# tangtang888/video-edge-ai-proxy

Measured on AMD Instinct MI355X. Metric: decoded FPS (whole node) + p50 VideoLatestImage latency, 256×1080p RTSP, higher is better.
Workload: dtype uint8 (BGR24 frames; bf16-capable consumer path)

## Files before the change

csrc/bind_codec.cpp:

```cpp
#include "bind_common.h"
#include "vep/avc.h"
#include "vep/codec.h"
#include "vep/hevc_dec.h"
#include "vep/hevc_kern.h"
#include "vep/synth.h"

struct CpuDecoder {
  StreamParser parser;
  MbUpdate upd;
  HostSurface surf;
  PictureInfo last;
  avc::Decoder avc;
  std::vector<HostSurface> slots;
  bool general = false;
  int target = 0;
  int coded = 0;
  bool fields_out = false;
  HostSurface woven;
  mutable HostSurface weave_tmp;
  const HostSurface& out() const { return general ? (fields_out ? woven : slots[size_t(target)]) : surf; }
  const HostSurface& frame_of(const avc::OutFrame& f) const {
    if (!f.fields) return slots[size_t(f.slot)];
    avc::weave_fields(slots[2 * size_t(f.slot)], slots[2 * size_t(f.slot) + 1], weave_tmp);
    return weave_tmp;
// ... 209 lines not shown
      .def_readwrite("weighted_b", &avc::AvcHighConfig::weighted_b)
      .def_readwrite("direct_spatial", &avc::AvcHighConfig::direct_spatial)
      .def_readwrite("scaling", &avc::AvcHighConfig::scaling)
      .def_readwrite("slices", &avc::AvcHighConfig::slices)
      .def_readwrite("deblock_idc", &avc::AvcHighConfig::deblock_idc)
      .def_readwrite("chroma_qp_offset", &avc::AvcHighConfig::chroma_qp_offset)
      .def_readwrite("second_chroma_qp_offset", &avc::AvcHighConfig::second_chroma_qp_offset)
      .def_readwrite("coverage", &avc::AvcHighConfig::coverage)
      .def_readwrite("interlaced", &avc::AvcHighConfig::interlaced)
      .def_readwrite("mono", &avc::AvcHighConfig::mono)
      .def_readwrite("fields", &avc::AvcHighConfig::fields)
      .def_readwrite("marking", &avc::AvcHighConfig::marking)
      .def_readwrite("objects", &avc::AvcHighConfig::objects)
      .def_readwrite("noise", &avc::AvcHighConfig::noise)
      .def_readwrite("temporal_noise", &avc::AvcHighConfig::temporal_noise)
      .def_readwrite("seed", &avc::AvcHighConfig::seed);
  py::class_<avc::AvcHighEncoder>(m, "AvcHighEncoder")
      .def(py::init<const avc::AvcHighConfig&>())
      .def("next", &avc::AvcHighEncoder::next, py::call_guard<py::gil_scoped_release>())
      .def("picture", [](const avc::AvcHighEncoder& e) { return surface_planes(e.reconstruction()); })
      .def("source", [](const avc::AvcHighEncoder& e) { return surface_planes(e.source()); })
      .def_property_readonly("last_pts", &avc::AvcHighEncoder::last_pts)
      .def_property_readonly("last_type", [](const avc::AvcHighEncoder& e) { return std::string(1, e.last_type()); })
      .def_property_readonly("last_display_index", &avc::AvcHighEncoder::last_display_index)
      .def_property_readonly("sps_nal", [](const avc::AvcHighEncoder& e) { return to_bytes(e.sps_nal().data(), e.sps_nal().size()); })
      .def_property_readonly("pps_nal", [](const avc::AvcHighEncoder& e) { return to_bytes(e.pps_nal().data(), e.pps_nal().size()); });

  py::class_<hevc::HevcEncConfig>(m, "HevcEncConfig")
      .def(py::init<>())
      .def_readwrite("width", &hevc::HevcEncConfig::width)
// ... 211 lines not shown
```

csrc/bind_codec_hooks.cpp:

```cpp
#include "bind_common.h"
#include "vep/avc.h"
#include "vep/avc_cavlc.h"
#include "vep/avc_recon.h"
#include "vep/cabac.h"
#include "vep/codec.h"
#include "vep/h264.h"
#include "vep/hevc_ctu.h"
#include "vep/hevc_dec.h"
#include "vep/hevc_kern.h"
#include "vep/synth.h"

struct XorShift {
  u64 x;
  XorShift(u64 seed, u64 salt) : x(seed * 0x9E3779B97F4A7C15ull + salt) {}
  u64 operator()() { return x ^= x << 13, x ^= x >> 7, x ^= x << 17; }
};

static std::vector<u8> rbsp_of(const std::string& nal) {
  std::vector<u8> r(nal.size());
  r.resize(ebsp_to_rbsp(reinterpret_cast<const u8*>(nal.data()), nal.size(), r.data()));
  return r;
}

void bind_codec_hooks(py::module_& m) {
// ... 317 lines not shown
      mbs += p->mbs.size();
      coefs += p->coefs.size();
      mvs += p->mvs.size();
      for (const avc::MbRec& m : p->mbs)
        if (m.kind != avc::kIPcm) nz += avc::coef_values(p->coefs.data(), m);
    }
    py::gil_scoped_acquire g;
    py::dict d;
    d["pictures"] = pics;
    d["mbs"] = mbs;
    d["coefs"] = coefs;
    d["nonzero"] = nz;
    d["mvs"] = mvs;
    return d;
  });
  m.def("hevc_record_stats", [](const std::vector<std::shared_ptr<AccessUnit>>& aus) {
    py::gil_scoped_release r;
    hevc::Decoder dec;
    dec.set_gpu_mode(true);
    u64 pics = 0, tus = 0, coefs = 0, nz = 0, pus = 0;
    for (const auto& au : aus) {
      dec.decode(*au);
      for (const auto& p : dec.take_gpu_pictures()) {
        ++pics;
        tus += p->tus.size();
        pus += p->pus.size();
        coefs += p->coefs.size();
        for (i16 c : p->coefs) nz += c != 0;
      }
    }
// ... 135 lines not shown
```

csrc/vep/avc.cpp:

```cpp
#include "avc.h"

#include <immintrin.h>

#include <algorithm>
#include <array>

#include "avc_cavlc.h"
#include "avc_internal.h"
#include "fanout.h"

namespace vep::avc {

using h264::Pps;
using h264::Sps;


void MbNeighbours::reset(int wmbs, int hmbs, bool ring) {
  w_ = wmbs;
  h_ = hmbs;
  cur_ = -1;
  run_slice_ = ~0u;
  run_start_ = 0;
  announced_ = 0;
  const size_t n = size_t(wmbs) * hmbs;
// ... 1402 lines not shown
      pi.coded_height = sps.coded_height();
      pi.width = sps.width();
      pi.height = sps.height();
      pi.crop_left = sps.crop_left;
      pi.crop_top = sps.crop_top;
      pi.pict_type = "PBISi"[sh.type()];
      pi.idr = sh.idr();
      pi.frame_num = sh.frame_num;
      pi.fps = sps.fps();
      pic->au.pts = au.pts;
      pic->au.dts = au.dts;
      pic->au.arrival_ms = au.arrival_ms;
      pic->au.keyframe = au.keyframe;
      pic->au.corrupt = au.corrupt;
      pic->au.tag = tag;
      nb_.reset(W, Hp, true);
      if (sh.field_pic) {
        const int fs = second_field ? pair_.slot : pick_slot();
        pic->target = 2 * fs + int(sh.bottom_field);
        if (!second_field) {
          pair_ = OpenPair{};
          pair_.open = true;
          pair_.slot = fs;
          pair_.frame_num = sh.frame_num;
          pair_.bottom = int(sh.bottom_field);
          pair_.ref = sh.nal_ref_idc != 0;
          pair_.boundary = sh.idr();
          pair_.hard = sh.idr() && (hard_flush || reorder_cur_ == 0);
          pair_.f.slot = fs;
          pair_.f.info = pic->info;
          pair_.f.au = pic->au;
// ... 322 lines not shown

void ColBuild::none(int mb) {
  const int per = col->corners ? 4 : 16;
  ColMotion::Blk* out = &col->b[size_t(mb) * size_t(per)];
  for (int k = 0; k < per; ++k) out[k] = ColMotion::Blk{{0, 0}, 0u, i8(-1)};
}

void ColBuild::store(int mb, const MbState& st) {
  if (is_intra(st.kind) || !uids) {
    none(mb);
    return;
  }
  static constexpr u8 kCorner[4] = {0, 3, 12, 15};
  const auto& lu = *uids;
  if (col->corners) {
    ColMotion::Blk out[4];
    for (int k = 0; k < 4; ++k) {
      const int l = st.ref[0][k] >= 0 ? 0 : 1;
      const int ri = st.ref[l][k];
      out[k] = ri < 0 ? ColMotion::Blk{{0, 0}, 0u, i8(-1)}
                      : ColMotion::Blk{{st.mv[l][kCorner[k]][0], st.mv[l][kCorner[k]][1]}, uid_tab[l][ri & 31], i8(ri)};
    }
    stream_words(&col->b[size_t(mb) * 4], out, sizeof out);
    return;
  }
  ColMotion::Blk* out = &col->b[size_t(mb) * 16];
  for (int blk = 0; blk < 16; ++blk) {
    const int b8 = ((blk >> 3) << 1) | ((blk & 3) >> 1);
    const int l = st.ref[0][b8] >= 0 ? 0 : 1;
    const int ri = st.ref[l][b8];
    if (ri < 0) {
      out[blk] = ColMotion::Blk{{0, 0}, 0u, i8(-1)};
      continue;
    }
    out[blk] = ColMotion::Blk{{st.mv[l][blk][0], st.mv[l][blk][1]},
                              size_t(ri) < lu[size_t(l)].size() ? lu[size_t(l)][size_t(ri)] : 0u, i8(ri)};
  }
}

std::shared_ptr<ColMotion> build_col_motion(const MbNeighbours& nb, int wmbs, int hmbs,
                                            const std::vector<std::array<std::vector<u32>, 2>>& slice_uids,
                                            bool corners, Recycler<ColMotion>* pool) {
  auto col = pool ? pool->acquire([](ColMotion&) {}) : std::make_shared<ColMotion>();
  col->wmbs = wmbs;
  col->hmbs = hmbs;
  col->corners = corners;
  const int per = corners ? 4 : 16;
  col->b.resize(size_t(wmbs) * hmbs * size_t(per));
  static constexpr u8 kCorner[4] = {0, 3, 12, 15};
  for (int mb = 0; mb < wmbs * hmbs; ++mb) {
    const MbState& st = nb.at(mb);
    ColMotion::Blk* out = &col->b[size_t(mb) * size_t(per)];
// ... 214 lines not shown
  const __m256i tl = _mm256_setr_epi32(0, 0, 2, 2, 0, 0, 2, 2);
  const u32 all = u32(_mm256_movemask_epi8(_mm256_and_si256(_mm256_cmpeq_epi32(a, v0), _mm256_cmpeq_epi32(b, v0))));
  const u32 q8 = u32(_mm256_movemask_epi8(_mm256_and_si256(_mm256_cmpeq_epi32(a, _mm256_permutevar8x32_epi32(a, tl)),
                                                           _mm256_cmpeq_epi32(b, _mm256_permutevar8x32_epi32(b, tl)))));
  return (all == 0xFFFFFFFFu ? 1u : 0u) | (q8 == 0xFFFFFFFFu ? 2u : 0u);
#else
  u32 v[16];
  std::memcpy(v, mv, sizeof v);
  bool u16 = true, u8x8 = true;
  for (int b = 1; b < 16; ++b) u16 &= v[b] == v[0];
  for (int b = 0; b < 16; ++b) u8x8 &= v[b] == v[((b >> 3) << 3) | (b & 2)];
  return (u16 ? 1u : 0u) | (u8x8 ? 2u : 0u);
#endif
}

static inline void store_motion(Picture& pic, MbRec& m, const MbState& s) {
  const int nl = (m.flags & kMbL1) ? 2 : 1;
  u32 u = 3;
  for (int l = 0; l < nl; ++l) u &= motion_uniformity(&s.mv[l][0][0]);
  m.flags |= (u & 1) ? kMbMv16 : ((u & 2) ? kMbMv8x8 : 0);
  m.mv = u32(pic.mvs.size());
  const int per = (u & 1) ? 2 : ((u & 2) ? 8 : 32);
  i16* out = pic.mvs.extend(size_t(per * nl));
  for (int l = 0; l < nl; ++l, out += per) {
    const i16* v = &s.mv[l][0][0];
    if (per == 2) {
      std::memcpy(out, v, 4);
    } else if (per == 8) {
      std::memcpy(out, v, 4);
      std::memcpy(out + 2, v + 4, 4);
      std::memcpy(out + 4, v + 16, 4);
      std::memcpy(out + 6, v + 20, 4);
    } else {
      std::memcpy(out, v, 64);
    }
  }
}

static inline void store_rec(MbRec* dst, const MbRec& m) {
  static_assert(sizeof(MbRec) % 8 == 0 && sizeof(ColMotion::Blk) * 4 % 8 == 0, "8-byte words");
  stream_words(dst, &m, sizeof(MbRec));
}

void store_skip_mb(Picture& pic, int mb, MbRec& m, const MbState& s) {
  m.coef = u32(pic.coefs.size());
  m.luma_coded = 0;
  m.chroma_coded = 0;
  m.wp = 0;
  m.res = kNoRes;
  store_motion(pic, m, s);
  ++pic.inter_mbs;
  if (!(m.dbk & 1)) pic.deblock = true;
  for (int k = 0; k < 4; ++k) {
    const int r0 = m.ref[k], r1 = m.ref1[k];
    VEP_CHECK((r0 != 0xFF || r1 != 0xFF) && (r0 == 0xFF || r0 < pic.dpb_slots) && (r1 == 0xFF || r1 < pic.dpb_slots) &&
                  (r1 == 0xFF || (m.flags & kMbL1)),
              "skipped macroblock reference slot outside the DPB");
  }
  VEP_CHECK(m.qp <= 51 + pic.qp_bias && m.qpc <= 51 + pic.qpc_bias && m.qpc2 <= 51 + pic.qpc_bias,
            "macroblock QP out of range");
  store_rec(&pic.mbs[size_t(mb)], m);
  if (pic.colb) pic.colb->store(mb, s);
}

void store_mb(Picture& pic, int mb, MbRec m, const MbState& s, const MbResidual* res, const u8* pcm,
              const WpEntry* wp) {
  m.coef = u32(pic.coefs.size());
  m.luma_coded = 0;
  m.chroma_coded = 0;
  if (m.kind == kIPcm) {
    VEP_CHECK(pcm, "I_PCM macroblock without samples");
    const size_t ns = pic.cf == 2 ? size_t(kPcmMaxSamples) : size_t(kPcmMbBytes);
    const size_t o = pic.coefs.size(), nb = pic.bd > 8 ? 2 * ns : ns;
    pic.coefs.resize(o + nb / 2);
    std::memcpy(pic.coefs.data() + o, pcm, nb);
  } else if (res && (res->luma | res->chroma)) {
    m.luma_coded = res->luma;
    m.chroma_coded = res->chroma;
    if (res->t8) m.flags |= kMbT8x8;
    const i16* grp[32];
    int ng = 0;
// ... 10 lines not shown
    for (int g = 0; g < ng; ++g) {
      mask[g] = nonzero_mask16(grp[g]);
      nv += __builtin_popcount(mask[g]);
    }
    const size_t o = pic.coefs.size();
    i16* out = pic.coefs.extend(size_t(ng + nv) + 8);
    std::memcpy(out, mask, size_t(ng) * sizeof(u16));
    i16* v = out + ng;
    for (int g = 0; g < ng; ++g) v = compact16(grp[g], mask[g], v);
    pic.coefs.resize(o + size_t(ng + nv));
  }
  m.mv = 0;
  m.wp = 0;
  m.flags &= u8(~(kMbMv8x8 | kMbMv16));
  if (m.kind == kSkip || m.kind == kInter) {
    store_motion(pic, m, s);
    if (wp && (m.flags & kMbWp)) {
      m.wp = u32(pic.wps.size());
      pic.wps.insert(pic.wps.end(), wp, wp + 4);
    } else {
      m.flags &= u8(~kMbWp);
    }
    ++pic.inter_mbs;
  } else if (m.kind == kIPcm) {
    ++pic.inter_mbs;
  } else {
    ++pic.intra_mbs;
  }
  m.res = is_intra(m.kind) && m.kind != kIPcm && (m.luma_coded | m.chroma_coded) ? u32(pic.intra_res++) : kNoRes;
  if (!(m.dbk & 1)) pic.deblock = true;
  validate_written_mb(pic, m);
// ... 356 lines not shown
```

csrc/vep/avc.h:

```cpp
#pragma once

#include <array>
#include <map>
#include <memory>

#include "hostmem.h"
#include "recycle.h"
#include "avc_recon.h"
#include "codec.h"

namespace vep::avc {

constexpr int kMaxDpbSlots = 34;

struct AuMeta {
  i64 pts = 0, dts = 0, arrival_ms = 0;
  i64 tag = 0;
  bool keyframe = false, corrupt = false;
};

struct OutFrame {
  int slot = -1;
  PictureInfo info;
  AuMeta au;
// ... 324 lines not shown
    return corners ? size_t(mb) * 4 + size_t(((blk >> 3) << 1) | ((blk & 3) >> 1)) : size_t(mb) * 16 + size_t(blk);
  }
};

struct ColBuild {
  ColMotion* col = nullptr;
  const std::array<std::vector<u32>, 2>* uids = nullptr;
  u32 uid_tab[2][32] = {};
  void set_uids(const std::array<std::vector<u32>, 2>* u) {
    uids = u;
    for (int l = 0; l < 2; ++l)
      for (size_t k = 0; k < 32; ++k) uid_tab[l][k] = u && k < (*u)[size_t(l)].size() ? (*u)[size_t(l)][k] : 0u;
  }
  void store(int mb, const MbState& st);
  void none(int mb);
};

struct RefPic {
  int slot = -1;
  int frame_num = 0;
  int frame_num_wrap = 0;
  bool long_term = false;
  int lt_idx = 0;
  int poc = 0;
  u32 uid = 0;
  std::shared_ptr<const ColMotion> col;
  u8 fields = 3;
  u8 lt_fields = 0;
  int poc_f[2] = {0, 0};
  u32 uid_f[2] = {0, 0};
// ... 55 lines not shown
  int cf_ = 1;
  bool have_idr_ = false;
  int pinned_slot_ = -1;
  int last_out_poc_ = 0;
  i64 last_out_epoch_ = -1;
  u32 epoch_ = 0;
  int adaptive_reorder_ = 0;
  int reorder_cur_ = 0;
  u32 next_uid_ = 1;
  int prev_poc_msb_ = 0, prev_poc_lsb_ = 0;
  int prev_frame_num_ = 0, prev_frame_num_offset_ = 0;
  bool prev_ref_mmco5_ = false;
  std::vector<std::vector<MbState>> spare_;
  struct SliceUnit;
  bool parallel_slices_ = true;
  std::vector<std::unique_ptr<SliceUnit>> units_;
  u64 parallel_slices_run_ = 0;
  bool field_mode_ = false;
  struct OpenPair {
    bool open = false;
    int slot = -1, frame_num = 0, bottom = 0;
    int poc[2] = {0, 0};
    bool ref = false, boundary = false, hard = false;
    u8 have = 0;
    OutFrame f;
  } pair_;
  void close_pair(Picture& pic);

 public:
  Decoder();
  ~Decoder();
  u64 parallel_slices_run() const { return parallel_slices_run_; }
  u64 mmco_ops[7] = {0, 0, 0, 0, 0, 0, 0};
  u64 list_mods = 0, long_term_marked = 0;
  u64 redundant_slices_skipped = 0;
};

void cpu_reconstruct(const Picture& pic, std::vector<HostSurface>& slots);
void weave_fields(const HostSurface& top, const HostSurface& bottom, HostSurface& frame);

struct MbLevels {
  int luma[16][16];
  int dc[16];
  int cdc[2][4];
  int cac[2][4][16];
  u16 lmask = 0;
  u8 cmask = 0;
// ... 9 lines not shown
      for (int b = 0; b < 4; ++b) {
        if (cdc[c][b]) dcmask |= u8(2 << c);
        for (int k = 0; k < 16; ++k)
          if (cac[c][b][k]) cmask |= u8(1u << (c * 4 + b));
      }
  }
};
struct MbResidual {
  i16 blk[32][16];
  i16 b8[4][64];
  u16 luma = 0;
  u16 chroma = 0;
  bool t8 = false;
};
void dequantize_mb(const MbLevels& lv, bool i16x16, int qp, int qpc, MbResidual& out);
void store_mb(Picture& pic, int mb, MbRec m, const MbState& s, const MbResidual* res, const u8* pcm,
              const WpEntry* wp = nullptr);
void store_skip_mb(Picture& pic, int mb, MbRec& m, const MbState& s);
void cpu_reconstruct_mb(const Picture& pic, int mb, std::vector<HostSurface>& slots);
void cpu_deblock(const Picture& pic, HostSurface& target);
void intra4x4_neighbours(const Picture& pic, int mb, int idx, const HostSurface& T, Intra4Nb& n);
void intra16_neighbours(const Picture& pic, int mb, const HostSurface& T, Intra16Nb& n);
void chroma_neighbours(const Picture& pic, int mb, int c, const HostSurface& T, IntraChromaNb& n);
void intra8x8_neighbours(const Picture& pic, int mb, int q, const HostSurface& T, int* f, bool& has_top,
                         bool& has_left);

class StreamEncoder {
 public:
  virtual ~StreamEncoder() = default;
  virtual std::shared_ptr<AccessUnit> next() = 0;
  virtual const HostSurface& reconstruction() const = 0;
  virtual const HostSurface& source() const = 0;
  virtual i64 last_pts() const = 0;
// ... 53 lines not shown
  int weighted_b = 0;
  bool direct_spatial = true;
  bool scaling = false;
  int slices = 1;
  int deblock_idc = 0;
  int chroma_qp_offset = 0, second_chroma_qp_offset = 0;
  bool coverage = false;
  bool interlaced = false;
  bool marking = false;
  bool fields = false;
  bool mono = false;
  int bit_depth = 8;
  int chroma_format = 1;
  int objects = 3;
  double noise = 3.0, temporal_noise = 0.0;
  u64 seed = 1;
};

class AvcHighEncoder : public StreamEncoder {
 public:
  explicit AvcHighEncoder(const AvcHighConfig& cfg);
  ~AvcHighEncoder() override;
  std::shared_ptr<AccessUnit> next() override;
  const HostSurface& reconstruction() const override;
  const HostSurface& source() const override;
  i64 last_pts() const override;
  i64 last_display_index() const;
  char last_type() const;
  const AvcHighConfig& config() const { return cfg_; }
  const std::vector<u8>& sps_nal() const override;
// ... 10 lines not shown
```

csrc/vep/avc_enc_high.cpp:

```cpp
#include <cmath>
#include <deque>
#include <map>

#include "avc.h"
#include "avc_internal.h"
#include "avc_scene.h"
#include "h264.h"

namespace vep::avc {

namespace {

struct Idct8Inverse {
  double inv[8][8];
  Idct8Inverse() {
    double m[8][8];
    for (int k = 0; k < 8; ++k) {
      int x[8] = {0, 0, 0, 0, 0, 0, 0, 0};
      x[k] = 1024;
      idct8_1d(x);
      for (int i = 0; i < 8; ++i) m[i][k] = x[i] / 1024.0;
    }
    double a[8][16];
    for (int i = 0; i < 8; ++i)
// ... 76 lines not shown
    int lt_idx = 0;
    u8 lt_fields = 0;
  };
  int max_lt_idx = -1;
  std::vector<Ref> dpb;
  struct Job {
    i64 disp;
    int type;
    bool ref;
    bool idr;
    int parity = -1;
  };
  std::deque<Job> plan;
  std::map<i64, HostSurface> sources;
  i64 next_disp = 0, gop_start = 0, rendered = -1, coded = 0;
  int prev_ref_fn = 0, idr_id = -1;
  u32 next_uid = 1;
  Picture pic;
  MbNeighbours nb;
  HostSurface recon, src_out;
  i64 last_disp = 0, last_pts = 0;
  char last_type = 'I';
  const HostSurface* cur_src = nullptr;
  bool fields = false;
  int ph = 0;
  HostSurface field_src;
  int pair_slot = -1, pair_fn = 0;
  int bd = 8, qpbd = 0;
  int cf = 1;
  const u8* scan4 = kZigzag4x4;
// ... 53 lines not shown
    pps.cabac = c.cabac;
    pps.bottom_field_pic_order = c.interlaced;
    pps.weighted_pred = c.weighted_p;
    pps.weighted_bipred_idc = c.weighted_b;
    pps.chroma_qp_index_offset = c.chroma_qp_offset;
    pps.second_chroma_qp_index_offset = c.second_chroma_qp_offset;
    pps.deblocking_filter_control = true;
    pps.transform_8x8_mode = c.t8x8;
    pps.scaling.flat();
    auto nal = [](const std::vector<u8>& rbsp, std::vector<u8>& out) { rbsp_to_ebsp(rbsp.data(), rbsp.size(), out); };
    nal(h264::write_sps(sps), sps_nal);
    nal(h264::write_pps(pps), pps_nal);
    ph = fields ? hpx / 2 : hpx;
    slots.resize((size_t(sps.max_num_ref_frames) + 2) * (fields ? 2 : 1));
    for (auto& s : slots) s.alloc(wpx, ph, bd, cf);
    scene.make(SceneConfig{c.width, c.height, wpx, hpx, c.objects, c.noise, c.temporal_noise, c.seed}, rng);
  }

  bool is_idr_pos(i64 d) const { return d == 0 || (d + cfg.idr_phase) % cfg.gop == 0; }

  const HostSurface& source_of(i64 d) {
    while (rendered < d) {
      ++rendered;
      if (rendered > 0) scene.advance();
      scene.render();
      scene.add_sensor_noise(rendered);
      if (bd > 8 || cf == 2) {
        HostSurface& w = sources[rendered];
        const HostSurface& s8 = scene.src;
        w.alloc(s8.coded_w, s8.coded_h, bd, cf);
        const int sh = bd - 8;
// ... 826 lines not shown
    const double dist = (e.poc - env.cur_poc) / 2.0;
    const int mx = mb % W, my = mb / W;
    auto cost = [&](int vx, int vy) {
      int s = 0;
      for (int i = 0; i < 16; i += 2)
        for (int j = 0; j < 16; j += 2) {
          const int x = mx * 16 + j, y = my * 16 + i;
          const int p = bd > 8 ? luma_qpel(R.y16.data(), wpx, wpx, ph, x + (vx >> 2), y + (vy >> 2), vx & 3, vy & 3, bd)
                               : luma_qpel(R.y.data(), wpx, wpx, ph, x + (vx >> 2), y + (vy >> 2), vx & 3, vy & 3);
          s += std::abs(S(x, y) - p);
        }
      return s * 4 + 4 * (std::abs(vx - pmv[0]) + std::abs(vy - pmv[1]));
    };
    std::vector<std::pair<int, int>> cand = {{0, 0}, {pmv[0], pmv[1]}};
    const double ys = fields ? 0.5 : 1.0;
    for (const Scene::Obj& o : scene.objs) {
      if (o.x > mx * 16 + 24 || o.x + o.w < mx * 16 - 8 || o.y * ys > my * 16 + 24 || (o.y + o.h) * ys < my * 16 - 8)
        continue;
      cand.push_back({int(std::lround(o.vx * 4 * dist)), int(std::lround(o.vy * ys * 4 * dist))});
    }
    best_sad = 1 << 30;
    for (auto [vx, vy] : cand) {
      const int c = cost(vx, vy);
      if (c < best_sad) {
        best_sad = c;
        best[0] = vx;
        best[1] = vy;
      }
    }
    for (int step : {4, 2, 1}) {
// ... 634 lines not shown
```

csrc/vep/avc_mb.cpp:

```cpp
#include <algorithm>
#include <memory>
#include <cstddef>
#include <cstring>

#include "avc_cabac.h"
#include "avc_cavlc.h"
#include "avc_internal.h"

namespace vep::avc {

namespace {

struct Dequant {
  int ls4[6][6][16];
  int ls8[2][6][64];
  explicit Dequant(const h264::ScalingLists& sl) {
    for (int l = 0; l < 6; ++l)
      for (int m = 0; m < 6; ++m)
        for (int k = 0; k < 16; ++k) {
          const int pos = kZigzag4x4[k];
          ls4[l][m][pos] = int(sl.l4[l][k]) * norm_adjust(m, pos >> 2, pos & 3);
        }
    for (int l = 0; l < 2; ++l)
      for (int m = 0; m < 6; ++m)
// ... 112 lines not shown
    auto cond = [&](int m) { return m >= 0 && !nb_.at(m).skip ? 1 : 0; };
    const int inc = cond(nb_.mb_at(mb, -1, 0)) + cond(nb_.mb_at(mb, 0, -1));
    return bins->mb_skip(type_ == h264::kB, inc, v) != 0;
  }

  void skip_mb(int mb, bool fresh) {
    MbState& s = nb_.at(mb);
    if (fresh) {
      s = MbState{};
      s.slice = u16(env_.slice);
      nb_.begin(mb);
    }
    s.kind = kSkip;
    s.skip = 1;
    s.qp = u8(qp_ + qpbd_);
    MbResidual res;
    res.luma = 0;
    res.chroma = 0;
    if (type_ == h264::kP) {
      s.ref[0][0] = s.ref[0][1] = s.ref[0][2] = s.ref[0][3] = 0;
      need_ref(0, 0);
      int mv[2];
      nb_.pskip_mv(mb, mv);
      for (auto& v : s.mv[0]) {
        v[0] = i16(mv[0]);
        v[1] = i16(mv[1]);
      }
    } else {
      s.direct16 = 1;
      s.direct8 = 0xF;
      if (fast_direct_) direct16_spatial(mb, s);
      else direct(mb, s, 0xF);
    }
    prev_qpd_nz = 0;
    if (!weighted_ && !kWrite) emit_skip(mb, s);
    else emit(mb, s, res, 0, 0, nullptr);
  }

  void coded_mb(int mb, bool fresh) {
    MbState& s = nb_.at(mb);
    if (fresh) {
      s = MbState{};
      s.slice = u16(env_.slice);
      nb_.begin(mb);
    } else if constexpr (!kWrite) {
      std::memset(static_cast<void*>(s.mv), 0, sizeof s.mv);
    }
    int mbt = read_mb_type(mb, kWrite ? want->mb_type : 0);
    int itype = -1;
    if (type_ == h264::kI) {
      itype = mbt;
// ... 587 lines not shown
          const int tx = (16384 + std::abs(td / 2)) / td;
          const int dsf = clip3i(-1024, 1023, (tb * tx + 32) >> 6);
          for (int k = 0; k < 2; ++k) {
            m0[k] = (dsf * mvc[k] + 128) >> 8;
            m1[k] = m0[k] - mvc[k];
          }
        }
        fill(0, b8, blk, clip3i(-32768, 32767, m0[0]), clip3i(-32768, 32767, m0[1]));
        fill(1, b8, blk, clip3i(-32768, 32767, m1[0]), clip3i(-32768, 32767, m1[1]));
      }
      s.ref[0][b8] = i8(r0);
      s.ref[1][b8] = 0;
    }
  }

  void direct16_spatial(int mb, MbState& s) {
    if (!dcol_) {
      VEP_CHECK(env_.list[1] && !env_.list[1]->empty() && (*env_.list[1])[0].slot >= 0,
                "direct prediction without a list-1 reference");
      const ListEntry& c1 = (*env_.list[1])[0];
      VEP_CHECK(c1.col && c1.col->wmbs == nb_.wmbs() && c1.col->hmbs == nb_.hmbs() && c1.col->corners,
                "colocated picture motion missing");
      dcol_ = c1.col;
      dcol_long_ = c1.long_term;
    }
    int ref[2], mvp[2][2];
    nb_.direct_spatial_both(ref, mvp);
    const bool zero = ref[0] < 0 && ref[1] < 0;
    if (zero) ref[0] = ref[1] = 0;
    u32 pv[2];
    for (int l = 0; l < 2; ++l) {
      if (ref[l] >= 0) need_ref(l, ref[l]);
      const bool use = ref[l] >= 0 && !zero;
      pv[l] = use ? (u32(u16(mvp[l][0])) | u32(u16(mvp[l][1])) << 16) : 0u;
      std::memset(s.ref[l], ref[l], 4);
    }
    const ColMotion::Blk* cb = &dcol_->b[size_t(mb) * 4];
    u32 v8[2][4];
    for (int b8 = 0; b8 < 4; ++b8) {
      const bool col_zero = !dcol_long_ && cb[b8].ref == 0 && cb[b8].mv[0] >= -1 && cb[b8].mv[0] <= 1 &&
                            cb[b8].mv[1] >= -1 && cb[b8].mv[1] <= 1;
      for (int l = 0; l < 2; ++l) v8[l][b8] = (ref[l] == 0 && col_zero) ? 0u : pv[l];
    }
    for (int l = 0; l < 2; ++l) {
      u32 row[2][4];
      for (int h = 0; h < 2; ++h) {
        row[h][0] = row[h][1] = v8[l][2 * h];
        row[h][2] = row[h][3] = v8[l][2 * h + 1];
      }
      u8* mv = reinterpret_cast<u8*>(&s.mv[l][0][0]);
      for (int y = 0; y < 4; ++y) std::memcpy(mv + 16 * y, row[y >> 1], 16);
    }
  }

  WpEntry weights(int r0, int r1) { return wp_entry(env_, r0, r1); }

  int cbf_luma_inc(int mb, int blk, bool intra) {
    auto cond = [&](int m, int nblk) -> int {
      if (m < 0) return intra ? 1 : 0;
      const MbState& n = nb_.at(m);
      if (n.kind == kIPcm) return 1;
      if (n.skip) return 0;
      if (!((n.cbp >> raster_b8(nblk)) & 1)) return 0;
      if (n.t8x8) return 1;
      return (n.cbf >> nblk) & 1;
    };
    const int bx = blk & 3, by = blk >> 2;
// ... 194 lines not shown
              const int k = nzp[j];
              const int pos = scan4_[k + 1];
              const int v = scale4(lv[k], dq_.ls4[lc][qpc[c] % 6][pos], qpc[c]);
              d[pos] = sat16(v);
              nz |= v != 0;
            }
          }
          if (nz) res.chroma |= u16(1u << (c * nbc + b));
        }
      }
    }
    if constexpr (!kCabac && !kWrite) VEP_CHECK(!br->overrun(), "slice data overrun");
  }

  void emit(int mb, const MbState& s, const MbResidual& res, int i16_mode, int chroma_mode, const u8* pcm) {
    MbRec m{};
    m.kind = s.kind;
    m.qp = u8(s.kind == kIPcm ? qpbd_ : s.qp);
    VEP_CHECK(m.qp < std::size(qpc_tab_[0]), "macroblock QP out of range");
    m.qpc = qpc_tab_[0][m.qp];
    m.qpc2 = qpc_tab_[1][m.qp];
    m.i16_mode = u8(i16_mode);
    m.chroma_mode = u8(chroma_mode);
    m.dbk = u8((sh_.disable_deblocking == 1 ? 1 : 0) | (sh_.disable_deblocking == 2 ? 2 : 0));
    m.alpha_off = i8(sh_.alpha_off);
    m.beta_off = i8(sh_.beta_off);
    m.slice = s.slice;
    m.flags = s.t8x8 && s.kind != kI8x8 ? kMbT8x8 : 0;
    if (s.kind == kI8x8) m.flags = kMbT8x8;
    bool l1 = false;
// ... 22 lines not shown
      for (int r = 0; r < 16; ++r) m.i4[r >> 1] |= u8(s.i4[r] << ((r & 1) * 4));
    if (s.kind == kI8x8)
      for (int b8 = 0; b8 < 4; ++b8) m.i4[b8 >> 1] |= u8(s.i4[(b8 & 1) * 2 + (b8 >> 1) * 8] << ((b8 & 1) * 4));
    WpEntry wp[4];
    bool use_wp = false;
    if (weighted_ && !is_intra(s.kind)) {
      for (int k = 0; k < 4; ++k) {
        wp[k] = weights(s.ref[0][k], s.ref[1][k]);
        const WpEntry& e = wp[k];
        for (int c = 0; c < 3; ++c)
          use_wp |= !(e.lwd[c] == 0 && e.w0[c] == 1 && e.w1[c] == 1 && e.o[c] == 0) &&
                    !(e.w0[c] == (1 << e.lwd[c]) && e.w1[c] == (1 << e.lwd[c]) && e.o[c] == 0);
      }
      if (use_wp) m.flags |= kMbWp;
    }
    store_mb(pic_, mb, m, s, &res, pcm, use_wp ? wp : nullptr);
  }

  void emit_skip(int mb, const MbState& s) {
    MbRec m{};
    m.kind = kSkip;
    m.qp = s.qp;
    VEP_CHECK(m.qp < std::size(qpc_tab_[0]), "macroblock QP out of range");
    m.qpc = qpc_tab_[0][m.qp];
    m.qpc2 = qpc_tab_[1][m.qp];
    m.dbk = u8((sh_.disable_deblocking == 1 ? 1 : 0) | (sh_.disable_deblocking == 2 ? 2 : 0));
    m.alpha_off = i8(sh_.alpha_off);
    m.beta_off = i8(sh_.beta_off);
    m.slice = s.slice;
    bool l1 = false;
    for (int k = 0; k < 4; ++k) {
      m.ref[k] = slot_[0][s.ref[0][k] + 1];
      m.ref1[k] = slot_[1][s.ref[1][k] + 1];
      l1 |= s.ref[1][k] >= 0;
    }
    m.flags = l1 ? kMbL1 : 0;
    nz8_ = 0;
    store_skip_mb(pic_, mb, m, s);
  }

  MbNeighbours& nb_;
  Picture& pic_;
  const SliceEnv& env_;
  const SliceHdr& sh_;
  const h264::Pps& pps_;
  const h264::Sps& sps_;
  const Dequant& dq_;
  const u8* scan4_;
  const u8* scan8_;
  int type_ = 0;
  int qp_ = 26;
  bool weighted_ = false, implicit_ = false;
  u16 nz8_ = 0;
  u8 slot_[2][33];
  u8 qpc_tab_[2][96];
  bool fast_direct_ = false;
  const ColMotion* dcol_ = nullptr;
  bool dcol_long_ = false;
};

}

WpEntry wp_entry(const SliceEnv& env, int r0, int r1) {
  const SliceHdr& sh = *env.sh;
  const bool implicit = sh.type() == h264::kB && env.pps->weighted_bipred_idc == 2;
  WpEntry e{};
  for (int c = 0; c < 3; ++c) {
    e.w0[c] = e.w1[c] = 1;
    e.o[c] = 0;
    e.lwd[c] = 0;
  }
  if (implicit) {
    if (r0 < 0 || r1 < 0) return e;
// ... 184 lines not shown
```

csrc/vep/avc_scene.h:

```cpp
#pragma once

#include <algorithm>
#include <cmath>

#include "codec.h"

namespace vep::avc {

struct Rng {
  u64 s;
  u64 next() {
    s ^= s << 13;
    s ^= s >> 7;
    s ^= s << 17;
    return s;
  }
  int uni(int n) { return int(next() % u64(n)); }
  bool chance(int pct) { return uni(100) < pct; }
};

inline u32 hash2(u32 x, u32 y, u32 seed) {
  u32 h = x * 0x8da6b343u ^ y * 0xd8163841u ^ seed * 0xcb1ab31fu;
  h ^= h >> 13;
  h *= 0x5bd1e995u;
// ... 35 lines not shown
  const int qbits = 15 + qp / 6 + extra_shift;
  const int f = (1 << qbits) / (intra ? 3 : 6);
  const long long a = (static_cast<long long>(w < 0 ? -w : w) * kMF[qp % 6][cls] + f) >> qbits;
  const int l = int(a > 2047 ? 2047 : a);
  return w < 0 ? -l : l;
}


struct SceneConfig {
  int width, height;
  int wpx, hpx;
  int objects;
  double noise;
  double temporal_noise;
  u64 seed;
};

class Scene {
 public:
  struct Obj {
    double x, y, vx, vy;
    int w, h;
    bool ellipse;
    double p1, p2, p3;
    int by, bu, bv;
  };
  HostSurface bg, src;
  std::vector<Obj> objs;

  void make(const SceneConfig& c, Rng& rng) {
// ... 30 lines not shown
      o.bu = 90 + rng.uni(80);
      o.bv = 90 + rng.uni(80);
      objs.push_back(o);
    }
  }

  bool inside(const Obj& o, double lx, double ly) const {
    if (lx < 0 || ly < 0 || lx >= o.w || ly >= o.h) return false;
    if (!o.ellipse) return true;
    const double dx = (lx - o.w / 2.0) / (o.w / 2.0), dy = (ly - o.h / 2.0) / (o.h / 2.0);
    return dx * dx + dy * dy <= 1.0;
  }

  void render() {
    const int wpx = cfg_.wpx;
    src.y = bg.y;
    src.uv = bg.uv;
    for (const Obj& o : objs) {
      const int x0 = std::max(0, int(std::floor(o.x))), y0 = std::max(0, int(std::floor(o.y)));
      const int x1 = std::min(cfg_.width, int(std::ceil(o.x + o.w)) + 1);
      const int y1 = std::min(cfg_.height, int(std::ceil(o.y + o.h)) + 1);
      for (int y = y0; y < y1; ++y)
        for (int x = x0; x < x1; ++x) {
          const double lx = x - o.x, ly = y - o.y;
          if (!inside(o, lx, ly)) continue;
          src.y[size_t(y) * wpx + x] =
              sat8(o.by + 50 * std::sin(lx * o.p1) * std::cos(ly * o.p2) + 25 * std::sin((lx + ly) * o.p3));
        }
      for (int y = y0 / 2; y < (y1 + 1) / 2; ++y)
        for (int x = x0 / 2; x < (x1 + 1) / 2; ++x) {
          const double lx = 2 * x - o.x, ly = 2 * y - o.y;
          if (!inside(o, lx, ly)) continue;
          src.uv[size_t(y) * wpx + 2 * x] = sat8(o.bu + 20 * std::sin(lx * o.p2));
          src.uv[size_t(y) * wpx + 2 * x + 1] = sat8(o.bv + 20 * std::cos(ly * o.p1));
        }
    }
  }

  void add_sensor_noise(i64 frame) {
    if (cfg_.temporal_noise <= 0) return;
    const u32 seed = u32(frame * 0x9E3779B1u) ^ u32(cfg_.seed);
    const int amp = int(cfg_.temporal_noise * 2) + 1;
    for (int y = 0; y < cfg_.hpx; ++y)
      for (int x = 0; x < cfg_.wpx; ++x) {
        u8& p = src.y[size_t(y) * cfg_.wpx + x];
        const int n = int(hash2(u32(x), u32(y), seed) % u32(amp)) - amp / 2;
        p = u8(std::min(255, std::max(0, p + n)));
      }
  }

  void advance() {
    for (Obj& o : objs) {
      o.x += o.vx;
      o.y += o.vy;
      if (o.x < -o.w / 2.0 || o.x + o.w / 2.0 > cfg_.width) o.vx = -o.vx;
      if (o.y < -o.h / 2.0 || o.y + o.h / 2.0 > cfg_.height) o.vy = -o.vy;
    }
  }

 private:
  SceneConfig cfg_{};
};

}
```

Baseline: 8315.

## Share uniform skip-MB motion vectors and short-circuit repeated skip records

In AVC parsing, consecutive skip macroblocks whose single 16x16 motion vector and references match the previous one now reuse its MV pool entry and MbRec instead of appending new data. The co-located motion store repeats cached corner blocks. Spatial direct prediction gains a fast path for when the three neighbours agree, and it reports whether the result is uniform. The change also adds a panned-scene option to the synthetic encoder and a motion audit hook for testing. All of this aims to cut per-MB store and bandwidth cost on static or panning content, at the risk of subtle correctness problems in direct prediction and shared MV offsets.

```diff
diff --git a/csrc/bind_codec.cpp b/csrc/bind_codec.cpp
--- a/csrc/bind_codec.cpp
+++ b/csrc/bind_codec.cpp
@@ -247,6 +247,8 @@
       .def_readwrite("objects", &avc::AvcHighConfig::objects)
       .def_readwrite("noise", &avc::AvcHighConfig::noise)
       .def_readwrite("temporal_noise", &avc::AvcHighConfig::temporal_noise)
+      .def_readwrite("pan_x", &avc::AvcHighConfig::pan_x)
+      .def_readwrite("pan_y", &avc::AvcHighConfig::pan_y)
       .def_readwrite("seed", &avc::AvcHighConfig::seed);
   py::class_<avc::AvcHighEncoder>(m, "AvcHighEncoder")
       .def(py::init<const avc::AvcHighConfig&>())
diff --git a/csrc/bind_codec_hooks.cpp b/csrc/bind_codec_hooks.cpp
--- a/csrc/bind_codec_hooks.cpp
+++ b/csrc/bind_codec_hooks.cpp
@@ -355,6 +355,108 @@
     d["mvs"] = mvs;
     return d;
   });
+  m.def("avc_motion_audit", [](const std::vector<std::shared_ptr<AccessUnit>>& aus) {
+    py::gil_scoped_release r;
+    avc::Decoder dec;
+    dec.keep_mb_state();
+    u64 inter = 0, mismatched = 0, outside = 0, pool = 0, per_mb = 0, shared = 0, b_pics = 0;
+    u64 after_intra = 0, after_l0 = 0, after_l1 = 0, after_bi = 0, row_cross = 0, agree_nonzero = 0;
+    u64 gran[3] = {0, 0, 0};
+    u64 ref1 = 0, slice_first_skips = 0;
+    for (const auto& au : aus) {
+      auto p = dec.parse(*au);
+      if (!p) continue;
+      const avc::MbNeighbours& nb = dec.mb_state();
+      b_pics += p->info.pict_type == 'B';
+      pool += p->mvs.size();
+      const int W = p->wmbs;
+      size_t fresh_end = 0;
+      auto is_inter = [](const avc::MbRec& m) { return m.kind == avc::kSkip || m.kind == avc::kInter; };
+      auto word16 = [&](const avc::MbRec& m, int l) -> u64 {
+        if (!(m.flags & avc::kMbMv16)) return ~u64(0);
+        u32 w;
+        std::memcpy(&w, &p->mvs[size_t(m.mv) + size_t(avc::mv_sub(m.flags, l, 0))], 4);
+        return w;
+      };
+      for (int mb = 0; mb < p->nmbs(); ++mb) {
+        const avc::MbRec& m = p->mbs[size_t(mb)];
+        if (!is_inter(m)) continue;
+        ++inter;
+        const int nl = (m.flags & avc::kMbL1) ? 2 : 1, per = avc::mv_per_list(m.flags);
+        per_mb += u64(per * nl);
+        ++gran[per == 2 ? 0 : (per == 8 ? 1 : 2)];
+        if (size_t(m.mv) + size_t(per * nl) > p->mvs.size()) {
+          ++outside;
+          continue;
+        }
+        if (size_t(m.mv) < fresh_end) ++shared;
+        fresh_end = std::max(fresh_end, size_t(m.mv) + size_t(per * nl));
+        const avc::MbState& s = nb.at(mb);
+        bool bad = false;
+        for (int l = 0; l < nl; ++l)
+          for (int blk = 0; blk < 16; ++blk) {
+            const i16* v = &p->mvs[size_t(m.mv) + size_t(avc::mv_sub(m.flags, l, blk))];
+            bad |= v[0] != s.mv[l][blk][0] || v[1] != s.mv[l][blk][1];
+          }
+        mismatched += bad;
+        for (int k = 0; k < 4; ++k) ref1 += s.ref[0][k] > 0 || s.ref[1][k] > 0;
+        if (m.kind != avc::kSkip) continue;
+        const int mx = mb % W;
+        const bool prev_same_slice = mb > 0 && p->mbs[size_t(mb) - 1].slice == m.slice;
+        if (!prev_same_slice) {
+          ++slice_first_skips;
+          continue;
+        }
+        const avc::MbRec& q = p->mbs[size_t(mb) - 1];
+        if (q.kind == avc::kSkip) {
+          row_cross += mx == 0;
+        } else if (!is_inter(q)) {
+          ++after_intra;
+        } else {
+          const bool l0 = q.ref[0] != 0xFF || q.ref[1] != 0xFF || q.ref[2] != 0xFF || q.ref[3] != 0xFF;
+          const bool l1 = q.ref1[0] != 0xFF || q.ref1[1] != 0xFF || q.ref1[2] != 0xFF || q.ref1[3] != 0xFF;
+          (l0 && l1 ? after_bi : (l1 ? after_l1 : after_l0)) += 1;
+        }
+        const int my = mb / W;
+        if (mx > 0 && my > 0 && p->info.pict_type == 'B') {
+          const int cn = mx + 1 < W ? mb - W + 1 : mb - W - 1;
+          const avc::MbRec* n3[3] = {&p->mbs[size_t(mb) - 1], &p->mbs[size_t(mb - W)], &p->mbs[size_t(cn)]};
+          bool agree = (m.flags & avc::kMbMv16) != 0;
+          u64 any = 0;
+          for (const avc::MbRec* n : n3) {
+            agree = agree && is_inter(*n) && n->slice == m.slice && (n->flags & avc::kMbL1) == (m.flags & avc::kMbL1) &&
+                    std::memcmp(n->ref, m.ref, 4) == 0 && std::memcmp(n->ref1, m.ref1, 4) == 0;
+            for (int l = 0; agree && l < nl; ++l) {
+              agree = word16(*n, l) == word16(m, l);
+              any |= word16(m, l);
+            }
+          }
+          agree_nonzero += agree && any != 0;
+        }
+      }
+    }
+    py::gil_scoped_acquire g;
+    py::dict d;
+    d["inter_mbs"] = inter;
+    d["mismatched"] = mismatched;
+    d["outside_pool"] = outside;
+    d["pool_entries"] = pool;
+    d["per_mb_entries"] = per_mb;
+    d["shared"] = shared;
+    d["b_pictures"] = b_pics;
+    d["mv16"] = gran[0];
+    d["mv8x8"] = gran[1];
+    d["mv4x4"] = gran[2];
+    d["ref_idx_above_0"] = ref1;
+    d["skip_first_in_slice"] = slice_first_skips;
+    d["skip_after_intra"] = after_intra;
+    d["skip_after_l0"] = after_l0;
+    d["skip_after_l1"] = after_l1;
+    d["skip_after_bi"] = after_bi;
+    d["skip_run_row_cross"] = row_cross;
+    d["skip_agreeing_nonzero"] = agree_nonzero;
+    return d;
+  });
   m.def("hevc_record_stats", [](const std::vector<std::shared_ptr<AccessUnit>>& aus) {
     py::gil_scoped_release r;
     hevc::Decoder dec;
diff --git a/csrc/vep/avc.cpp b/csrc/vep/avc.cpp
--- a/csrc/vep/avc.cpp
+++ b/csrc/vep/avc.cpp
@@ -1440,7 +1440,7 @@
       pic->au.keyframe = au.keyframe;
       pic->au.corrupt = au.corrupt;
       pic->au.tag = tag;
-      nb_.reset(W, Hp, true);
+      nb_.reset(W, Hp, !keep_state_);
       if (sh.field_pic) {
         const int fs = second_field ? pair_.slot : pick_slot();
         pic->target = 2 * fs + int(sh.bottom_field);
@@ -1793,14 +1793,13 @@
   static constexpr u8 kCorner[4] = {0, 3, 12, 15};
   const auto& lu = *uids;
   if (col->corners) {
-    ColMotion::Blk out[4];
     for (int k = 0; k < 4; ++k) {
       const int l = st.ref[0][k] >= 0 ? 0 : 1;
       const int ri = st.ref[l][k];
-      out[k] = ri < 0 ? ColMotion::Blk{{0, 0}, 0u, i8(-1)}
-                      : ColMotion::Blk{{st.mv[l][kCorner[k]][0], st.mv[l][kCorner[k]][1]}, uid_tab[l][ri & 31], i8(ri)};
-    }
-    stream_words(&col->b[size_t(mb) * 4], out, sizeof out);
+      last[k] = ri < 0 ? ColMotion::Blk{{0, 0}, 0u, i8(-1)}
+                       : ColMotion::Blk{{st.mv[l][kCorner[k]][0], st.mv[l][kCorner[k]][1]}, uid_tab[l][ri & 31], i8(ri)};
+    }
+    stream_words(&col->b[size_t(mb) * 4], last, sizeof last);
     return;
   }
   ColMotion::Blk* out = &col->b[size_t(mb) * 16];
@@ -1815,6 +1814,11 @@
     out[blk] = ColMotion::Blk{{st.mv[l][blk][0], st.mv[l][blk][1]},
                               size_t(ri) < lu[size_t(l)].size() ? lu[size_t(l)][size_t(ri)] : 0u, i8(ri)};
   }
+}
+
+void ColBuild::repeat(int mb, const MbState& st) {
+  if (col->corners && uids) stream_words(&col->b[size_t(mb) * 4], last, sizeof last);
+  else store(mb, st);
 }
 
 std::shared_ptr<ColMotion> build_col_motion(const MbNeighbours& nb, int wmbs, int hmbs,
@@ -2059,11 +2063,30 @@
 #endif
 }
 
-static inline void store_motion(Picture& pic, MbRec& m, const MbState& s) {
+static inline void store_motion(Picture& pic, MbRec& m, const MbState& s, MvShare* share = nullptr,
+                                bool may_share = false, bool uniform16 = false) {
   const int nl = (m.flags & kMbL1) ? 2 : 1;
   u32 u = 3;
-  for (int l = 0; l < nl; ++l) u &= motion_uniformity(&s.mv[l][0][0]);
+  if (!uniform16)
+    for (int l = 0; l < nl; ++l) u &= motion_uniformity(&s.mv[l][0][0]);
   m.flags |= (u & 1) ? kMbMv16 : ((u & 2) ? kMbMv8x8 : 0);
+  if (share) {
+    if (u & 1) {
+      u32 w0, w1 = 0;
+      std::memcpy(&w0, &s.mv[0][0][0], 4);
+      if (nl == 2) std::memcpy(&w1, &s.mv[1][0][0], 4);
+      const u64 words = u64(w0) | u64(w1) << 32;
+      if (may_share && share->nl == u32(nl) && share->words == words) {
+        m.mv = share->off;
+        return;
+      }
+      share->off = u32(pic.mvs.size());
+      share->nl = u32(nl);
+      share->words = words;
+    } else {
+      share->nl = 0;
+    }
+  }
   m.mv = u32(pic.mvs.size());
   const int per = (u & 1) ? 2 : ((u & 2) ? 8 : 32);
   i16* out = pic.mvs.extend(size_t(per * nl));
@@ -2087,13 +2110,13 @@
   stream_words(dst, &m, sizeof(MbRec));
 }
 
-void store_skip_mb(Picture& pic, int mb, MbRec& m, const MbState& s) {
+void store_skip_mb(Picture& pic, int mb, MbRec& m, const MbState& s, MvShare* share, bool uniform16) {
   m.coef = u32(pic.coefs.size());
   m.luma_coded = 0;
   m.chroma_coded = 0;
   m.wp = 0;
   m.res = kNoRes;
-  store_motion(pic, m, s);
+  store_motion(pic, m, s, share, true, uniform16);
   ++pic.inter_mbs;
   if (!(m.dbk & 1)) pic.deblock = true;
   for (int k = 0; k < 4; ++k) {
@@ -2108,8 +2131,14 @@
   if (pic.colb) pic.colb->store(mb, s);
 }
 
+void store_skip_repeat(Picture& pic, int mb, const MbRec& m, const MbState& s) {
+  ++pic.inter_mbs;
+  store_rec(&pic.mbs[size_t(mb)], m);
+  if (pic.colb) pic.colb->repeat(mb, s);
+}
+
 void store_mb(Picture& pic, int mb, MbRec m, const MbState& s, const MbResidual* res, const u8* pcm,
-              const WpEntry* wp) {
+              const WpEntry* wp, MvShare* share) {
   m.coef = u32(pic.coefs.size());
   m.luma_coded = 0;
   m.chroma_coded = 0;
@@ -2150,7 +2179,7 @@
   m.wp = 0;
   m.flags &= u8(~(kMbMv8x8 | kMbMv16));
   if (m.kind == kSkip || m.kind == kInter) {
-    store_motion(pic, m, s);
+    store_motion(pic, m, s, share, (s.skip | s.direct16) != 0);
     if (wp && (m.flags & kMbWp)) {
       m.wp = u32(pic.wps.size());
       pic.wps.insert(pic.wps.end(), wp, wp + 4);
diff --git a/csrc/vep/avc.h b/csrc/vep/avc.h
--- a/csrc/vep/avc.h
+++ b/csrc/vep/avc.h
@@ -362,6 +362,8 @@
   }
   void store(int mb, const MbState& st);
   void none(int mb);
+  void repeat(int mb, const MbState& st);
+  ColMotion::Blk last[4] = {};
 };
 
 struct RefPic {
@@ -447,6 +449,7 @@
   std::vector<std::vector<MbState>> spare_;
   struct SliceUnit;
   bool parallel_slices_ = true;
+  bool keep_state_ = false;
   std::vector<std::unique_ptr<SliceUnit>> units_;
   u64 parallel_slices_run_ = 0;
   bool field_mode_ = false;
@@ -464,6 +467,11 @@
   Decoder();
   ~Decoder();
   u64 parallel_slices_run() const { return parallel_slices_run_; }
+  void keep_mb_state() {
+    keep_state_ = true;
+    parallel_slices_ = false;
+  }
+  const MbNeighbours& mb_state() const { return nb_; }
   u64 mmco_ops[7] = {0, 0, 0, 0, 0, 0, 0};
   u64 list_mods = 0, long_term_marked = 0;
   u64 redundant_slices_skipped = 0;
@@ -503,9 +511,16 @@
   bool t8 = false;
 };
 void dequantize_mb(const MbLevels& lv, bool i16x16, int qp, int qpc, MbResidual& out);
+struct MvShare {
+  u32 off = 0;
+  u32 nl = 0;
+  u64 words = 0;
+};
 void store_mb(Picture& pic, int mb, MbRec m, const MbState& s, const MbResidual* res, const u8* pcm,
-              const WpEntry* wp = nullptr);
-void store_skip_mb(Picture& pic, int mb, MbRec& m, const MbState& s);
+              const WpEntry* wp = nullptr, MvShare* share = nullptr);
+void store_skip_mb(Picture& pic, int mb, MbRec& m, const MbState& s, MvShare* share = nullptr,
+                   bool uniform16 = false);
+void store_skip_repeat(Picture& pic, int mb, const MbRec& m, const MbState& s);
 void cpu_reconstruct_mb(const Picture& pic, int mb, std::vector<HostSurface>& slots);
 void cpu_deblock(const Picture& pic, HostSurface& target);
 void intra4x4_neighbours(const Picture& pic, int mb, int idx, const HostSurface& T, Intra4Nb& n);
@@ -589,6 +604,7 @@
   int chroma_format = 1;
   int objects = 3;
   double noise = 3.0, temporal_noise = 0.0;
+  double pan_x = 0, pan_y = 0;
   u64 seed = 1;
 };
 
diff --git a/csrc/vep/avc_enc_high.cpp b/csrc/vep/avc_enc_high.cpp
--- a/csrc/vep/avc_enc_high.cpp
+++ b/csrc/vep/avc_enc_high.cpp
@@ -114,6 +114,7 @@
   std::deque<Job> plan;
   std::map<i64, HostSurface> sources;
   i64 next_disp = 0, gop_start = 0, rendered = -1, coded = 0;
+  double pan[2] = {0, 0};
   int prev_ref_fn = 0, idr_id = -1;
   u32 next_uid = 1;
   Picture pic;
@@ -197,7 +198,10 @@
     ph = fields ? hpx / 2 : hpx;
     slots.resize((size_t(sps.max_num_ref_frames) + 2) * (fields ? 2 : 1));
     for (auto& s : slots) s.alloc(wpx, ph, bd, cf);
-    scene.make(SceneConfig{c.width, c.height, wpx, hpx, c.objects, c.noise, c.temporal_noise, c.seed}, rng);
+    scene.make(SceneConfig{c.width, c.height, wpx, hpx, c.objects, c.noise, c.temporal_noise, c.seed, c.pan_x, c.pan_y},
+               rng);
+    pan[0] = c.pan_x;
+    pan[1] = c.pan_y;
   }
 
   bool is_idr_pos(i64 d) const { return d == 0 || (d + cfg.idr_phase) % cfg.gop == 0; }
@@ -1054,6 +1058,8 @@
     };
     std::vector<std::pair<int, int>> cand = {{0, 0}, {pmv[0], pmv[1]}};
     const double ys = fields ? 0.5 : 1.0;
+    if (pan[0] != 0 || pan[1] != 0)
+      cand.push_back({int(std::lround(pan[0] * 4 * dist)), int(std::lround(pan[1] * ys * 4 * dist))});
     for (const Scene::Obj& o : scene.objs) {
       if (o.x > mx * 16 + 24 || o.x + o.w < mx * 16 - 8 || o.y * ys > my * 16 + 24 || (o.y + o.h) * ys < my * 16 - 8)
         continue;
diff --git a/csrc/vep/avc_mb.cpp b/csrc/vep/avc_mb.cpp
--- a/csrc/vep/avc_mb.cpp
+++ b/csrc/vep/avc_mb.cpp
@@ -150,9 +150,7 @@
     s.kind = kSkip;
     s.skip = 1;
     s.qp = u8(qp_ + qpbd_);
-    MbResidual res;
-    res.luma = 0;
-    res.chroma = 0;
+    bool uniform16 = false;
     if (type_ == h264::kP) {
       s.ref[0][0] = s.ref[0][1] = s.ref[0][2] = s.ref[0][3] = 0;
       need_ref(0, 0);
@@ -162,15 +160,22 @@
         v[0] = i16(mv[0]);
         v[1] = i16(mv[1]);
       }
+      uniform16 = true;
     } else {
       s.direct16 = 1;
       s.direct8 = 0xF;
-      if (fast_direct_) direct16_spatial(mb, s);
+      if (fast_direct_) uniform16 = direct16_spatial(mb, s);
       else direct(mb, s, 0xF);
     }
     prev_qpd_nz = 0;
-    if (!weighted_ && !kWrite) emit_skip(mb, s);
-    else emit(mb, s, res, 0, 0, nullptr);
+    if (!weighted_ && !kWrite) {
+      emit_skip(mb, s, uniform16);
+    } else {
+      MbResidual res;
+      res.luma = 0;
+      res.chroma = 0;
+      emit(mb, s, res, 0, 0, nullptr);
+    }
   }
 
   void coded_mb(int mb, bool fresh) {
@@ -788,7 +793,7 @@
     }
   }
 
-  void direct16_spatial(int mb, MbState& s) {
+  bool direct16_spatial(int mb, MbState& s) {
     if (!dcol_) {
       VEP_CHECK(env_.list[1] && !env_.list[1]->empty() && (*env_.list[1])[0].slot >= 0,
                 "direct prediction without a list-1 reference");
@@ -798,33 +803,79 @@
       dcol_ = c1.col;
       dcol_long_ = c1.long_term;
     }
-    int ref[2], mvp[2][2];
-    nb_.direct_spatial_both(ref, mvp);
-    const bool zero = ref[0] < 0 && ref[1] < 0;
-    if (zero) ref[0] = ref[1] = 0;
+    int ref[2];
     u32 pv[2];
+    if (!agreeing_neighbours(mb, ref, pv)) {
+      int mvp[2][2];
+      nb_.direct_spatial_both(ref, mvp);
+      for (int l = 0; l < 2; ++l) {
+        if (ref[l] >= 0) need_ref(l, ref[l]);
+        pv[l] = ref[l] >= 0 ? (u32(u16(mvp[l][0])) | u32(u16(mvp[l][1])) << 16) : 0u;
+      }
+    }
+    if (ref[0] < 0 && ref[1] < 0) {
+      ref[0] = ref[1] = 0;
+      need_ref(0, 0);
+      need_ref(1, 0);
+    }
+    std::memset(s.ref[0], ref[0], 4);
+    std::memset(s.ref[1], ref[1], 4);
+    u32 cz = 0;
+    if (((ref[0] == 0 && pv[0] != 0) || (ref[1] == 0 && pv[1] != 0)) && !dcol_long_) {
+      const ColMotion::Blk* cb = &dcol_->b[size_t(mb) * 4];
+      for (int b8 = 0; b8 < 4; ++b8)
+        cz |= u32(cb[b8].ref == 0 && cb[b8].mv[0] >= -1 && cb[b8].mv[0] <= 1 && cb[b8].mv[1] >= -1 &&
+                  cb[b8].mv[1] <= 1)
+              << b8;
+    }
+    if (cz == 0 || cz == 0xF) {
+      for (int l = 0; l < 2; ++l) {
+        u32 w[16];
+        std::fill(std::begin(w), std::end(w), (cz && ref[l] == 0) ? 0u : pv[l]);
+        std::memcpy(static_cast<void*>(s.mv[l]), w, sizeof w);
+      }
+      return true;
+    }
     for (int l = 0; l < 2; ++l) {
-      if (ref[l] >= 0) need_ref(l, ref[l]);
-      const bool use = ref[l] >= 0 && !zero;
-      pv[l] = use ? (u32(u16(mvp[l][0])) | u32(u16(mvp[l][1])) << 16) : 0u;
-      std::memset(s.ref[l], ref[l], 4);
-    }
-    const ColMotion::Blk* cb = &dcol_->b[size_t(mb) * 4];
-    u32 v8[2][4];
-    for (int b8 = 0; b8 < 4; ++b8) {
-      const bool col_zero = !dcol_long_ && cb[b8].ref == 0 && cb[b8].mv[0] >= -1 && cb[b8].mv[0] <= 1 &&
-                            cb[b8].mv[1] >= -1 && cb[b8].mv[1] <= 1;
-      for (int l = 0; l < 2; ++l) v8[l][b8] = (ref[l] == 0 && col_zero) ? 0u : pv[l];
-    }
-    for (int l = 0; l < 2; ++l) {
+      u32 v8[4];
+      for (int b8 = 0; b8 < 4; ++b8) v8[b8] = (ref[l] == 0 && ((cz >> b8) & 1)) ? 0u : pv[l];
       u32 row[2][4];
       for (int h = 0; h < 2; ++h) {
-        row[h][0] = row[h][1] = v8[l][2 * h];
-        row[h][2] = row[h][3] = v8[l][2 * h + 1];
+        row[h][0] = row[h][1] = v8[2 * h];
+        row[h][2] = row[h][3] = v8[2 * h + 1];
       }
       u8* mv = reinterpret_cast<u8*>(&s.mv[l][0][0]);
       for (int y = 0; y < 4; ++y) std::memcpy(mv + 16 * y, row[y >> 1], 16);
     }
+    return false;
+  }
+
+  bool agreeing_neighbours(int mb, int ref[2], u32 pv[2]) const {
+    const int a = nb_.mb_at(mb, -1, 0), b = nb_.mb_at(mb, 0, -1);
+    if ((a | b) < 0) return false;
+    int c = nb_.mb_at(mb, 16, -1), cblk = 12;
+    if (c < 0) {
+      c = nb_.mb_at(mb, -1, -1);
+      cblk = 15;
+    }
+    if (c < 0) return false;
+    const MbState &sa = nb_.at(a), &sb = nb_.at(b), &sc = nb_.at(c);
+    if (is_intra(sa.kind) || is_intra(sb.kind) || is_intra(sc.kind)) return false;
+    const int c8 = cblk == 12 ? 2 : 3;
+    for (int l = 0; l < 2; ++l) {
+      const int r = sa.ref[l][1];
+      if (sb.ref[l][2] != r || sc.ref[l][c8] != r) return false;
+      ref[l] = r;
+      pv[l] = 0;
+      if (r < 0) continue;
+      u32 va, vb, vc;
+      std::memcpy(&va, sa.mv[l][3], 4);
+      std::memcpy(&vb, sb.mv[l][12], 4);
+      std::memcpy(&vc, sc.mv[l][cblk], 4);
+      if (va != vb || va != vc) return false;
+      pv[l] = va;
+    }
+    return true;
   }
 
   WpEntry weights(int r0, int r1) { return wp_entry(env_, r0, r1); }
@@ -1049,6 +1100,7 @@
   }
 
   void emit(int mb, const MbState& s, const MbResidual& res, int i16_mode, int chroma_mode, const u8* pcm) {
+    rep_ok_ = false;
     MbRec m{};
     m.kind = s.kind;
     m.qp = u8(s.kind == kIPcm ? qpbd_ : s.qp);
@@ -1101,10 +1153,23 @@
       }
       if (use_wp) m.flags |= kMbWp;
     }
-    store_mb(pic_, mb, m, s, &res, pcm, use_wp ? wp : nullptr);
-  }
-
-  void emit_skip(int mb, const MbState& s) {
+    store_mb(pic_, mb, m, s, &res, pcm, use_wp ? wp : nullptr, kWrite ? nullptr : &share_);
+  }
+
+  void emit_skip(int mb, const MbState& s, bool uniform16) {
+    u32 r0, r1, w0, w1;
+    std::memcpy(&r0, s.ref[0], 4);
+    std::memcpy(&r1, s.ref[1], 4);
+    std::memcpy(&w0, s.mv[0][0], 4);
+    std::memcpy(&w1, s.mv[1][0], 4);
+    const bool any_l1 = (~r1 & 0x80808080u) != 0;
+    const u64 words = u64(w0) | (any_l1 ? u64(w1) << 32 : 0);
+    if (rep_ok_ && uniform16 && r0 == rep_ref_[0] && r1 == rep_ref_[1] && words == share_.words &&
+        s.qp == rep_rec_.qp) {
+      nz8_ = 0;
+      store_skip_repeat(pic_, mb, rep_rec_, s);
+      return;
+    }
     MbRec m{};
     m.kind = kSkip;
     m.qp = s.qp;
@@ -1123,7 +1188,11 @@
     }
     m.flags = l1 ? kMbL1 : 0;
     nz8_ = 0;
-    store_skip_mb(pic_, mb, m, s);
+    store_skip_mb(pic_, mb, m, s, &share_, uniform16);
+    rep_ok_ = uniform16;
+    rep_rec_ = m;
+    rep_ref_[0] = r0;
+    rep_ref_[1] = r1;
   }
 
   MbNeighbours& nb_;
@@ -1144,6 +1213,10 @@
   bool fast_direct_ = false;
   const ColMotion* dcol_ = nullptr;
   bool dcol_long_ = false;
+  MvShare share_;
+  bool rep_ok_ = false;
+  MbRec rep_rec_{};
+  u32 rep_ref_[2] = {0, 0};
 };
 
 }
diff --git a/csrc/vep/avc_scene.h b/csrc/vep/avc_scene.h
--- a/csrc/vep/avc_scene.h
+++ b/csrc/vep/avc_scene.h
@@ -73,6 +73,7 @@
   double noise;
   double temporal_noise;
   u64 seed;
+  double pan_x = 0, pan_y = 0;
 };
 
 class Scene {
@@ -133,8 +134,12 @@
 
   void render() {
     const int wpx = cfg_.wpx;
-    src.y = bg.y;
-    src.uv = bg.uv;
+    if (cfg_.pan_x != 0 || cfg_.pan_y != 0) {
+      render_panned_background();
+    } else {
+      src.y = bg.y;
+      src.uv = bg.uv;
+    }
     for (const Obj& o : objs) {
       const int x0 = std::max(0, int(std::floor(o.x))), y0 = std::max(0, int(std::floor(o.y)));
       const int x1 = std::min(cfg_.width, int(std::ceil(o.x + o.w)) + 1);
@@ -156,6 +161,20 @@
     }
   }
 
+  void render_panned_background() {
+    const int wpx = cfg_.wpx, hpx = cfg_.hpx;
+    const int sx = 2 * int(std::lround(cfg_.pan_x * double(frame_) / 2)), sy = 2 * int(std::lround(cfg_.pan_y * double(frame_) / 2));
+    auto wrap = [](int v, int n) { return ((v % n) + n) % n; };
+    for (int y = 0; y < hpx; ++y)
+      for (int x = 0; x < wpx; ++x)
+        src.y[size_t(y) * wpx + x] = bg.y[size_t(wrap(y - sy, hpx)) * wpx + wrap(x - sx, wpx)];
+    for (int y = 0; y < hpx / 2; ++y)
+      for (int x = 0; x < wpx / 2; ++x)
+        for (int c = 0; c < 2; ++c)
+          src.uv[size_t(y) * wpx + 2 * x + c] =
+              bg.uv[size_t(wrap(y - sy / 2, hpx / 2)) * wpx + 2 * wrap(x - sx / 2, wpx / 2) + c];
+  }
+
   void add_sensor_noise(i64 frame) {
     if (cfg_.temporal_noise <= 0) return;
     const u32 seed = u32(frame * 0x9E3779B1u) ^ u32(cfg_.seed);
@@ -169,6 +188,7 @@
   }
 
   void advance() {
+    ++frame_;
     for (Obj& o : objs) {
       o.x += o.vx;
       o.y += o.vy;
@@ -179,6 +199,7 @@
 
  private:
   SceneConfig cfg_{};
+  i64 frame_ = 0;
 };
 
 }
```

Result: faster. 8785 (median of 5 runs) (+5.6%).
